# JiehongLin/SAM-6D

Hardware: AMD Instinct MI355X
Metric: RGB-D frames/sec (SAM-6D per-frame hot path: SAM ViT-H encoder + ISM scoring + PEM) (higher is better)
Workload: dtype bf16 (SAM ViT-H: 87 % of the step) + f16 (PEM ViT-B feature extractor) + f32 (ISM scoring, PEM point transformer and pose solvers); 1 GPU; LM-O single object: 32 frames/step/GPU, 640x480 RGB-D -> 1024^2 SAM input, P=128 proposals x 42 templates (scored in groups of 8 frames), 1 instance/frame, 2048 pts (PEM batch 32); sam_frames_per_launch_group=16, pem_vit_dtype=fp16 (set by bench.py; the library default is fp32)

## Files before the change

sam6d_amd/csrc/s6d_attn_win16.h:

```cpp
#pragma once
#include "s6d_attn_common.h"

namespace S6D_ATTN_NS {

#ifndef S6D_WIN16_STREAM
#define S6D_WIN16_STREAM 1
#endif
#ifndef S6D_WIN16_KSWZ
#define S6D_WIN16_KSWZ 1
#endif

template <int HD>
struct RelFrags {
  union { uint4 u; bf16x8 v; } rh[2][Cfg<HD>::KS], rw[2][Cfg<HD>::KS];
  __device__ __forceinline__ void load(const AttnParams &p, int lane) {
    using C = Cfg<HD>;
    const int g = lane >> 4, c = lane & 15;
#pragma unroll
    for (int jt = 0; jt < 2; ++jt)
#pragma unroll
      for (int ks = 0; ks < C::KS; ++ks) {
        rh[jt][ks].u = *reinterpret_cast<const uint4 *>(p.rel_h + (size_t)(jt * 16 + c) * C::HDP + ks * 32 + g * 8);
        rw[jt][ks].u = *reinterpret_cast<const uint4 *>(p.rel_w + (size_t)(jt * 16 + c) * C::HDP + ks * 32 + g * 8);
      }
  }
};

constexpr int W16_LT = 36;

template <int HD, int NR, int SRC>
__device__ __forceinline__ void win16_tables(const RelFrags<HD> &rf, int S, int qy0, int rstride,
                                             const bf16x8 (*qf)[Cfg<HD>::KS], float *tab, float (*twr)[4],
                                             float (*thv)[16], int lane) {
  using C = Cfg<HD>;
  const int g = lane >> 4, c = lane & 15;
#pragma unroll
  for (int n = 0; n < NR; ++n) {
    const int qy = min(qy0 + n * rstride, S - 1);
    f32x4 ah[2], aw[2];
#pragma unroll
    for (int jt = 0; jt < 2; ++jt) {
      ah[jt] = f32x4{0.f, 0.f, 0.f, 0.f};
      aw[jt] = f32x4{0.f, 0.f, 0.f, 0.f};
#pragma unroll
      for (int ks = 0; ks < C::KS; ++ks) {
        aw[jt] = S6D_ATTN_MFMA16(rf.rw[jt][ks].v, qf[n][ks], aw[jt]);
        ah[jt] = S6D_ATTN_MFMA16(rf.rh[jt][ks].v, qf[n][ks], ah[jt]);
      }
    }
#pragma unroll
    for (int jt = 0; jt < 2; ++jt)
      *reinterpret_cast<float4 *>(tab + c * W16_LT + jt * 16 + g * 4) =
          make_float4(aw[jt][0] * kLog2e, aw[jt][1] * kLog2e, aw[jt][2] * kLog2e, aw[jt][3] * kLog2e);
    S6D_WAVE_RENDEZVOUS();
#pragma unroll
    for (int r = 0; r < 4; ++r) {
      const int kx = g * 4 + r;
      const float v = tab[c * W16_LT + min(max(c - kx + S - 1, 0), 31)];
      twr[n][r] = (kx < S && c < S) ? v : -1e30f;
    }
    S6D_WAVE_RENDEZVOUS();
#pragma unroll
    for (int jt = 0; jt < 2; ++jt)
      *reinterpret_cast<float4 *>(tab + c * W16_LT + jt * 16 + g * 4) =
          make_float4(ah[jt][0] * kLog2e, ah[jt][1] * kLog2e, ah[jt][2] * kLog2e, ah[jt][3] * kLog2e);
    S6D_WAVE_RENDEZVOUS();
#pragma unroll
    for (int ky = 0; ky < SRC; ++ky) {
      const float v = tab[c * W16_LT + min(max(qy - ky + S - 1, 0), 31)];
      thv[n][ky] = ky < S ? v : -1e30f;
    }
    S6D_WAVE_RENDEZVOUS();
  }
}

struct Win16NoMid {
  __device__ __forceinline__ void operator()() const {}
};
template <int HD, int NS, int SRC, bool EXACT, int KROWT = Cfg<HD>::KROW, bool KSWZ = false, class MID = Win16NoMid>
__device__ __forceinline__ void win16_pass(const AttnParams &p, const u16 *Kl, const u16 *Vl, int S, int SR, int b,
                                           int wy, int wx, int head, int qy0, int rstride,
                                           const bf16x8 (&qf)[NS][Cfg<HD>::KS], const float (*twr)[4],
                                           const float (*thv)[16], int lane, MID mid = MID()) {
  using C = Cfg<HD>;
  const int g = lane >> 4, c = lane & 15;
  const int Cc = p.nh * HD;
  float sp[NS][SRC][4], m[NS];
#pragma unroll
  for (int n = 0; n < NS; ++n) m[n] = -1e29f;
  f32x4 cb[NS];
  {
    const float inv = 1.0f / p.scale_log2;
#pragma unroll
    for (int n = 0; n < NS; ++n)
#pragma unroll
      for (int r = 0; r < 4; ++r) cb[n][r] = twr[n][r] * inv;
  }
  bf16x8 kf[2][C::KS];
  const int gk = KSWZ ? (g ^ kswz(c)) : g;
  auto kload = [&](int ky, bf16x8 (&dst)[C::KS]) {
    const int kyc = EXACT ? ky : min(ky, SR - 1);
#pragma unroll
    for (int ks = 0; ks < C::KS; ++ks) {
      dst[ks] = *reinterpret_cast<const bf16x8 *>(Kl + (kyc * 16 + c) * KROWT + ks * 32 + gk * 8);
      if (KROWT < C::HDP && ks * 32 + 32 > HD && ks * 32 + g * 8 >= HD) {
        union { bf16x8 v; uint4 u; } z;
        z.u = make_uint4(0, 0, 0, 0);
        dst[ks] = z.v;
      }
    }
  };
  kload(0, kf[0]);
#pragma unroll
  for (int ky = 0; ky < SRC; ++ky) {
    if (ky + 1 < SRC) kload(ky + 1, kf[(ky + 1) & 1]);
    f32x4 acc[NS];
#pragma unroll
    for (int n = 0; n < NS; ++n) acc[n] = cb[n];
#pragma unroll
    for (int ks = 0; ks < C::KS; ++ks)
#pragma unroll
      for (int n = 0; n < NS; ++n)
        acc[n] = S6D_ATTN_MFMA16(kf[ky & 1][ks], qf[n][ks], acc[n]);
#pragma unroll
    for (int n = 0; n < NS; ++n) {
#pragma unroll
      for (int r = 0; r < 4; ++r) sp[n][ky][r] = acc[n][r];
      const float mk = __builtin_fmaf(fmaxf(fmaxf(acc[n][0], acc[n][1]), fmaxf(acc[n][2], acc[n][3])), p.scale_log2, thv[n][ky]);
      m[n] = fmaxf(m[n], mk);
    }
  }
#pragma unroll
  for (int n = 0; n < NS; ++n) {
    m[n] = fmaxf(m[n], __shfl_xor(m[n], 16));
    m[n] = fmaxf(m[n], __shfl_xor(m[n], 32));
  }
  f32x4 oacc[NS][C::DT], lacc[NS];
#pragma unroll
  for (int n = 0; n < NS; ++n) {
    lacc[n] = f32x4{0.f, 0.f, 0.f, 0.f};
#pragma unroll
    for (int dt = 0; dt < C::DT; ++dt) oacc[n][dt] = f32x4{0.f, 0.f, 0.f, 0.f};
  }
  union { bf16x8 v; u16 hh[8]; } ones;
#pragma unroll
  for (int i = 0; i < 8; ++i) ones.hh[i] = S6D_ATTN_ONE;
#pragma unroll
  for (int u = 0; u < SRC; u += 2) {
    if (u == ((SRC / 2 + 1) & ~1)) {
      __builtin_amdgcn_sched_barrier(0);
      mid();
      __builtin_amdgcn_sched_barrier(0);
    }
    if (EXACT || u < SR) {
      union { bf16x8 v; s16x4 q[2]; } va[C::DT];
      const u16 *vrow = Vl + (u * 16 + g * 4 + (c >> 2)) * C::VROW + (c & 3) * 4;
#pragma unroll
      for (int dt = 0; dt < C::DT; ++dt) {
        va[dt].q[0] = __builtin_amdgcn_ds_read_tr16_b64_v4i16((S6D_LDS(s16x4) *)(vrow + dt * 16));
        va[dt].q[1] = __builtin_amdgcn_ds_read_tr16_b64_v4i16((S6D_LDS(s16x4) *)(vrow + 16 * C::VROW + dt * 16));
      }
      union { bf16x8 v; u16 hh[8]; } pb[NS];
#pragma unroll
      for (int n = 0; n < NS; ++n)
#pragma unroll
        for (int h = 0; h < 2; ++h) {
          const float nb = thv[n][u + h] - m[n];
          for (int r = 0; r < 4; ++r) pb[n].hh[h * 4 + r] = f2bf(fast_exp2(__builtin_fmaf(sp[n][u + h][r], p.scale_log2, nb)));
        }
#pragma unroll
      for (int n = 0; n < NS; ++n) lacc[n] = S6D_ATTN_MFMA16(ones.v, pb[n].v, lacc[n]);
#pragma unroll
      for (int dt = 0; dt < C::DT; ++dt)
#pragma unroll
        for (int n = 0; n < NS; ++n)
          oacc[n][dt] = S6D_ATTN_MFMA16(va[dt].v, pb[n].v, oacc[n][dt]);
    }
  }
#pragma unroll
  for (int n = 0; n < NS; ++n) {
    const int qy = qy0 + n * rstride;
    const int y = wy * p.ws + qy, x = wx * p.ws + c;
    if ((qy < S) && c < S && (y < p.H) && (x < p.W)) {
      const float inv = 1.0f / lacc[n][0];
      u16 *dst = p.out + ((size_t)(b * p.H + y) * p.W + x) * (size_t)Cc + head * HD;
#pragma unroll
      for (int dt = 0; dt < C::DT; ++dt) {
        union { uint2 u2; u16 hh[4]; } o;
#pragma unroll
        for (int r = 0; r < 4; ++r) o.hh[r] = f2bf(oacc[n][dt][r] * inv);
        *reinterpret_cast<uint2 *>(dst + dt * 16 + g * 4) = o.u2;
      }
    }
  }
}

template <int HD, int SRC, int KROWT, bool KSWZ, class NEXTQ, class THISQ>
__device__ __forceinline__ void win16_pass_stream(const AttnParams &p, const u16 *Kl, const u16 *Vl, int S, int b, int wy, int wx,
                                                  int head, int qy0, int rstride, const bf16x8 (&qf)[2][Cfg<HD>::KS],
                                                  const float (*twr)[4], const float (*thv)[16], int lane, NEXTQ next_q, THISQ this_q) {
  using C = Cfg<HD>;
  constexpr int NS = 2;
  static_assert(SRC % 2 == 0 && SRC >= 4, "whole 32-key steps");
  const int g = lane >> 4, c = lane & 15;
  const int Cc = p.nh * HD;
  const int gk = KSWZ ? (g ^ kswz(c)) : g;
  f32x4 cb[NS];
  {
    const float inv = 1.0f / p.scale_log2;
#pragma unroll
    for (int n = 0; n < NS; ++n)
#pragma unroll
      for (int r = 0; r < 4; ++r) cb[n][r] = twr[n][r] * inv;
  }
  bf16x8 kf[2][C::KS];
  auto kload = [&](int ky, bf16x8 (&dst)[C::KS]) __attribute__((always_inline)) {
#pragma unroll
    for (int ks = 0; ks < C::KS; ++ks) {
      dst[ks] = *reinterpret_cast<const bf16x8 *>(Kl + (ky * 16 + c) * KROWT + ks * 32 + gk * 8);
      if (KROWT < C::HDP && ks * 32 + 32 > HD && ks * 32 + g * 8 >= HD) {
        union { bf16x8 v; uint4 u; } z;
        z.u = make_uint4(0, 0, 0, 0);
        dst[ks] = z.v;
      }
    }
  };
  auto scores = [&](const bf16x8 (&k)[C::KS], f32x4 (&acc)[NS]) __attribute__((always_inline)) {
#pragma unroll
    for (int n = 0; n < NS; ++n) acc[n] = cb[n];
#pragma unroll
    for (int ks = 0; ks < C::KS; ++ks)
#pragma unroll
      for (int n = 0; n < NS; ++n) acc[n] = S6D_ATTN_MFMA16(k[ks], qf[n][ks], acc[n]);
  };
  f32x4 s0[NS], s1[NS];
  kload(0, kf[0]);
  kload(1, kf[1]);
  scores(kf[0], s0);
  scores(kf[1], s1);
  float m[NS];
#pragma unroll
  for (int n = 0; n < NS; ++n) {
    const float m0 = __builtin_fmaf(fmaxf(fmaxf(s0[n][0], s0[n][1]), fmaxf(s0[n][2], s0[n][3])), p.scale_log2, thv[n][0]);
    const float m1 = __builtin_fmaf(fmaxf(fmaxf(s1[n][0], s1[n][1]), fmaxf(s1[n][2], s1[n][3])), p.scale_log2, thv[n][1]);
    float v = fmaxf(fmaxf(m0, m1), -1e29f);
    v = fmaxf(v, __shfl_xor(v, 16));
    v = fmaxf(v, __shfl_xor(v, 32));
    m[n] = v;
  }
  union { bf16x8 v; u16 hh[8]; } ones;
#pragma unroll
  for (int i = 0; i < 8; ++i) ones.hh[i] = S6D_ATTN_ONE;
  f32x4 oacc[NS][C::DT], lacc[NS];
  int round = 0;
  for (;;) {
#pragma unroll
    for (int n = 0; n < NS; ++n) {
      lacc[n] = f32x4{0.f, 0.f, 0.f, 0.f};
#pragma unroll
      for (int dt = 0; dt < C::DT; ++dt) oacc[n][dt] = f32x4{0.f, 0.f, 0.f, 0.f};
    }
#pragma unroll
    for (int u = 0; u < SRC; u += 2) {
      if (u > 0 || round > 0) {
        kload(u, kf[0]);
        kload(u + 1, kf[1]);
        scores(kf[0], s0);
        scores(kf[1], s1);
      }
      if (u == SRC - 2 && round == 0) {
        __builtin_amdgcn_sched_barrier(0);
        next_q();
        __builtin_amdgcn_sched_barrier(0);
      }
      union { bf16x8 v; s16x4 q[2]; } va[C::DT];
      const u16 *vrow = Vl + (u * 16 + g * 4 + (c >> 2)) * C::VROW + (c & 3) * 4;
#pragma unroll
      for (int dt = 0; dt < C::DT; ++dt) {
        va[dt].q[0] = __builtin_amdgcn_ds_read_tr16_b64_v4i16((S6D_LDS(s16x4) *)(vrow + dt * 16));
        va[dt].q[1] = __builtin_amdgcn_ds_read_tr16_b64_v4i16((S6D_LDS(s16x4) *)(vrow + 16 * C::VROW + dt * 16));
      }
      union { bf16x8 v; u16 hh[8]; } pb[NS];
#pragma unroll
      for (int n = 0; n < NS; ++n) {
        const float nb0 = thv[n][u] - m[n], nb1 = thv[n][u + 1] - m[n];
#pragma unroll
        for (int r = 0; r < 4; ++r) {
          pb[n].hh[r] = f2bf(fast_exp2(__builtin_fmaf(s0[n][r], p.scale_log2, nb0)));
          pb[n].hh[4 + r] = f2bf(fast_exp2(__builtin_fmaf(s1[n][r], p.scale_log2, nb1)));
        }
      }
#pragma unroll
      for (int n = 0; n < NS; ++n) lacc[n] = S6D_ATTN_MFMA16(ones.v, pb[n].v, lacc[n]);
#pragma unroll
      for (int dt = 0; dt < C::DT; ++dt)
#pragma unroll
        for (int n = 0; n < NS; ++n) oacc[n][dt] = S6D_ATTN_MFMA16(va[dt].v, pb[n].v, oacc[n][dt]);
    }
    bool any_bad = false;
#pragma unroll
    for (int n = 0; n < NS; ++n) {
      const int qy = qy0 + n * rstride;
      int ovf = 0;
#pragma unroll
      for (int dt = 0; dt < C::DT; ++dt)
#pragma unroll
        for (int r = 0; r < 4; ++r) ovf |= !(fabsf(oacc[n][dt][r]) < kNoMaxFinite);
      ovf |= __shfl_xor(ovf, 16);
      ovf |= __shfl_xor(ovf, 32);
      const bool bad = (qy < S) && (c < S) && (!(lacc[n][0] < kNoMaxSumLimit) || ovf);
      m[n] = bad ? m[n] + 96.0f : m[n];
      any_bad |= bad;
    }
    if (!__any(any_bad) || round >= 40) break;
    if (round == 0) this_q();
    ++round;
  }
  if (round > 0) next_q();
#pragma unroll
  for (int n = 0; n < NS; ++n) {
    const int qy = qy0 + n * rstride;
    const int y = wy * p.ws + qy, x = wx * p.ws + c;
    if ((qy < S) && c < S && (y < p.H) && (x < p.W)) {
      const float inv = 1.0f / lacc[n][0];
      u16 *dst = p.out + ((size_t)(b * p.H + y) * p.W + x) * (size_t)Cc + head * HD;
#pragma unroll
      for (int dt = 0; dt < C::DT; ++dt) {
        union { uint2 u2; u16 hh[4]; } o;
#pragma unroll
        for (int r = 0; r < 4; ++r) o.hh[r] = f2bf(oacc[n][dt][r] * inv);
        *reinterpret_cast<uint2 *>(dst + dt * 16 + g * 4) = o.u2;
      }
    }
  }
}

template <int HD, int WAVES>
__global__ __launch_bounds__(WAVES * 64) void attn_window16_kernel(AttnParams p) {
  using C = Cfg<HD>;
  S6D_DYN_LDS(smem);
  const int S = p.S, SR = (S + 1) & ~1;
  u16 *Kl = reinterpret_cast<u16 *>(smem);
  u16 *Vl = Kl + (size_t)SR * 16 * C::KROW;
  float *tabs = reinterpret_cast<float *>(Vl + (size_t)SR * 16 * C::VROW);
  const int tid = threadIdx.x, wave = tid >> 6, lane = tid & 63;
  const int g = lane >> 4, c = lane & 15;
  float *tab = tabs + (size_t)wave * 16 * W16_LT;

  WinItem item;
  item.decode(p, blockIdx.x);
  const int head = item.head, wx = item.wx, wy = item.wy, b = item.b;
  const int Cc = p.nh * HD;
  constexpr int MAXROWS = 2;
  static_assert(2 * WAVES >= 16, "two rows per wave must cover 16 query rows");
  bf16x8 qfa[MAXROWS][C::KS];
#pragma unroll
  for (int i = 0; i < MAXROWS; ++i) {
    const int qy = wave + i * WAVES;
    const int y = wy * p.ws + qy, x = wx * p.ws + c;
    const bool qwin = c < S && qy < S, qimg = qwin && (y < p.H) && (x < p.W);
#pragma unroll
    for (int ks = 0; ks < C::KS; ++ks) {
      union { uint4 u; bf16x8 v; } t;
      const int d0 = ks * 32 + g * 8;
      const int dc = d0 < HD ? d0 : HD - 8;
      const size_t tokc = (size_t)(b * p.H + min(y, p.H - 1)) * p.W + min(x, p.W - 1);
      const u16 *src = qimg ? qkv_at(p, tokc, 0, head) + dc : p.qkv_bias + head * HD + dc;
      t.u = *reinterpret_cast<const uint4 *>(src);
      if (!(qwin && d0 < HD)) t.u = make_uint4(0, 0, 0, 0);
      qfa[i][ks] = t.v;
    }
  }
  RelFrags<HD> rf;
  rf.load(p, lane);
  constexpr int UN = 10;
  const int total = SR * 16 * (C::KPARTS + C::VPARTS);
  uint4 sv[UN];
  u16 *sdst[UN];
  auto issue = [&](int i0) {
#pragma unroll
    for (int n = 0; n < UN; ++n) {
      const int i = i0 + n * WAVES * 64;
      const int iq = min(i, total - 1);
      const bool isv = iq >= SR * 16 * C::KPARTS;
      const int ii = isv ? iq - SR * 16 * C::KPARTS : iq;
      const int parts = isv ? C::VPARTS : C::KPARTS;
      const int slot = ii / parts, part = ii - slot * parts;
      const int ky = slot >> 4, kx = slot & 15;
      const int y = wy * p.ws + ky, x = wx * p.ws + kx;
      sdst[n] = (i < total) ? (isv ? Vl + slot * C::VROW + part * 8 : Kl + slot * C::KROW + part * 8) : nullptr;
      const bool img = (y < p.H) && (x < p.W);
      const int dc = part * 8 < HD ? part * 8 : HD - 8;
      const size_t tokc = (size_t)(b * p.H + min(y, p.H - 1)) * p.W + min(x, p.W - 1);
      const int sel = (isv ? 2 : 1) * Cc + head * HD + dc;
      const u16 *src = img ? qkv_at(p, tokc, isv ? 2 : 1, head) + dc : p.qkv_bias + sel;
      sv[n] = *reinterpret_cast<const uint4 *>(src);
      if (!(ky < S && kx < S && part * 8 < HD)) sv[n] = make_uint4(0, 0, 0, 0);
    }
  };
  auto commit = [&]() {
#pragma unroll
    for (int n = 0; n < UN; ++n)
      if (sdst[n]) *reinterpret_cast<uint4 *>(sdst[n]) = sv[n];
  };
  const bool stage = !(kAbl & 1);
  if (stage) issue(tid);
  float twr[MAXROWS][4], thv[MAXROWS][16];
  if (!(kAbl & 2)) {
    if (S > WAVES) {
      if (S == 14)
        win16_tables<HD, 2, 14>(rf, S, wave, WAVES, qfa, tab, twr, thv, lane);
      else
        win16_tables<HD, 2, 16>(rf, S, wave, WAVES, qfa, tab, twr, thv, lane);
    } else if (wave < S) {
      win16_tables<HD, 1, 8>(rf, S, wave, WAVES, qfa, tab, twr, thv, lane);
    }
  }
  if (stage) {
    commit();
    for (int i0 = tid + UN * WAVES * 64; i0 < total; i0 += UN * WAVES * 64) {
      issue(i0);
      commit();
    }
  }
  __syncthreads();

  if (S <= WAVES) {
    if (wave < S && !(kAbl & 2)) {
      const bf16x8 (&q1)[1][C::KS] = reinterpret_cast<const bf16x8 (&)[1][C::KS]>(qfa[0]);
      win16_pass<HD, 1, 8, false>(p, Kl, Vl, S, SR, b, wy, wx, head, wave, WAVES, q1, twr, thv, lane);
    }
  } else if (!(kAbl & 2)) {
    static_assert(MAXROWS >= 2 || WAVES >= 16, "row bookkeeping");
    const bf16x8 (&q2)[2][C::KS] = reinterpret_cast<const bf16x8 (&)[2][C::KS]>(qfa[0]);
    if (S == 14) {
      win16_pass<HD, 2, 14, true>(p, Kl, Vl, S, SR, b, wy, wx, head, wave, WAVES, q2, twr, thv, lane);
    } else
      win16_pass<HD, 2, 16, false>(p, Kl, Vl, S, SR, b, wy, wx, head, wave, WAVES, q2, twr, thv, lane);
  }
}


template <int HD, bool S14>
__global__ __launch_bounds__(512) void attn_window16p_kernel(AttnParams p, int nitems) {
  using C = Cfg<HD>;
  constexpr int WAVES = 8;
  constexpr int KROWT = HD + 8, KCH = KROWT / 8, VCH = C::VROW / 8;
  S6D_DYN_LDS(smem);
  const int S = p.S, SR = (S + 1) & ~1;
  const int kchunks = SR * 16 * KCH, vchunks = SR * 16 * VCH;
  const int kinstr = (kchunks + 63) >> 6, vinstr = (vchunks + 63) >> 6;
  const int kbytes = kinstr << 10, bufbytes = kbytes + (vinstr << 10);
  u16 *relh = reinterpret_cast<u16 *>(smem + 2 * bufbytes);
  u16 *relw = relh + 32 * C::HDP;
  const int tid = threadIdx.x, wave = __builtin_amdgcn_readfirstlane(tid >> 6), lane = tid & 63;
  const int g = lane >> 4, c = lane & 15;
  const int Cc = p.nh * HD;
  constexpr int RCH = C::HDP / 8;
  for (int i = tid; i < 2 * 32 * RCH; i += 512) {
    const bool w = i >= 32 * RCH;
    const int ii = w ? i - 32 * RCH : i;
    const int row = ii / RCH, ch = ii - row * RCH;
    reinterpret_cast<uint4 *>(w ? relw : relh)[row * RCH + (ch ^ ((row >> 2) & 3))] = reinterpret_cast<const uint4 *>(w ? p.rel_w : p.rel_h)[ii];
  }

  constexpr int MAXI = S14 ? 5 : 6;
  static_assert(((S14 ? 14 : 16) * 16 * (KCH > VCH ? KCH : VCH) + 63) / 64 <= WAVES * MAXI,
                "attn_window16p_kernel: K / V image has more DMA pieces than the unrolled slots (raise MAXI)");
  unsigned kvc[MAXI];
  {
#pragma unroll
    for (int i = 0; i < MAXI; ++i) {
      unsigned both = 0;
#pragma unroll
      for (int which = 1; which <= 2; ++which) {
        const int rowch = which == 1 ? KCH : VCH, nch = which == 1 ? kchunks : vchunks;
        const int k = wave + i * WAVES;
        const int j = min((k << 6) + lane, nch - 1);
        const int slot = j / rowch, pp = j - slot * rowch;
        const int ky = slot >> 4, kx = slot & 15;
        const int part = (S6D_WIN16_KSWZ && which == 1 && pp * 8 < HD) ? pp ^ kswz(kx) : pp;
        const bool inwin = ky < S && kx < S && part * 8 < HD;
        const unsigned v = (unsigned)(ky & 15) | ((unsigned)kx << 4) | ((unsigned)part << 8) | ((unsigned)inwin << 12);
        both |= which == 1 ? v : v << 16;
      }
      kvc[i] = both;
    }
  }
  auto stage_image = [&](const WinItem &it, int which, char *dst_base) __attribute__((always_inline)) {
    const int ninstr = which == 1 ? kinstr : vinstr;
    const int y0 = it.wy * p.ws, x0 = it.wx * p.ws, bH = it.b * p.H;
    const u16 *base = qkv_at(p, 0, which, it.head);
    const u16 *bias_base = p.qkv_bias + which * Cc + it.head * HD;
#pragma unroll
    for (int i = 0; i < MAXI; ++i) {
      const int k = wave + i * WAVES;
      if (k < ninstr) {
        unsigned cc = which == 1 ? kvc[i] : kvc[i] >> 16;
        S6D_PIN(cc);
        const int ky = (int)(cc & 15u), kx = (int)((cc >> 4) & 15u), po = min((int)((cc >> 8) & 15u) * 8, HD - 8);
        const int y = y0 + ky, x = x0 + kx;
        const bool img = (y < p.H) && (x < p.W);
        const unsigned tok = (unsigned)(bH + min(y, p.H - 1)) * (unsigned)p.W + (unsigned)min(x, p.W - 1);
        const u16 *s_img = base + (size_t)tok * (size_t)p.tok_stride + po;
        const u16 *src = img ? s_img : bias_base + po;
        const void *sp = (cc >> 12) & 1u ? (const void *)src : (const void *)&g_attn_zero16;
        S6D_LDS(char) *dst = (S6D_LDS(char) *)dst_base + (k << 10);
        lds_dma16_m0(sp, dst);
      }
    }
  };
  constexpr int MAXROWS = 2;
  bf16x8 qfa[MAXROWS][C::KS];
  auto load_q = [&](const WinItem &it, bool raw, bf16x8 (&qdst)[MAXROWS][C::KS]) __attribute__((always_inline)) {
#pragma unroll
    for (int i = 0; i < MAXROWS; ++i) {
      const int qy = wave + i * WAVES;
      const int y = it.wy * p.ws + qy, x = it.wx * p.ws + c;
      const bool qwin = c < S && qy < S, qimg = qwin && (y < p.H) && (x < p.W);
#pragma unroll
      for (int ks = 0; ks < C::KS; ++ks) {
        union { uint4 u; bf16x8 v; } t;
        const int d0 = ks * 32 + g * 8;
        const int dc = d0 < HD ? d0 : HD - 8;
        const size_t tokc = (size_t)(it.b * p.H + min(y, p.H - 1)) * p.W + min(x, p.W - 1);
        const u16 *src = qimg ? qkv_at(p, tokc, 0, it.head) + dc : p.qkv_bias + it.head * HD + dc;
        t.u = *reinterpret_cast<const uint4 *>(src);
        if (!raw && !(qwin && d0 < HD)) t.u = make_uint4(0, 0, 0, 0);
        qdst[i][ks] = t.v;
      }
    }
  };
  auto mask_q = [&]() __attribute__((always_inline)) {
#pragma unroll
    for (int i = 0; i < MAXROWS; ++i) {
      const bool qwin = c < S && wave + i * WAVES < S;
#pragma unroll
      for (int ks = 0; ks < C::KS; ++ks) {
        union { uint4 u; bf16x8 v; } t;
        t.v = qfa[i][ks];
        if (!(qwin && ks * 32 + g * 8 < HD)) t.u = make_uint4(0, 0, 0, 0);
        qfa[i][ks] = t.v;
      }
    }
  };

  WinItem cur, nxt;
  int id = blockIdx.x;
  cur.decode(p, id);
  load_q(cur, false, qfa);
  stage_image(cur, 1, smem);
  stage_image(cur, 2, smem + kbytes);
  S6D_VMCNT(0);
  __syncthreads();
  int buf = 0;
  long long wtk[8] = {0, 0, 0, 0, 0, 0, 0, 0}, wsum[6] = {0, 0, 0, 0, 0, 0};
  for (; id < nitems; id += gridDim.x) {
    char *cb = smem + buf * bufbytes, *nb = smem + (buf ^ 1) * bufbytes;
    const bool more = id + (int)gridDim.x < nitems;
    S6D_TICK(wtk, 0);
    if (more) {
      nxt.decode(p, id + gridDim.x);
      stage_image(nxt, 1, nb);
    }
    float twr[MAXROWS][4], thv[MAXROWS][16];
    {
      RelFrags<HD> rf;
#pragma unroll
      for (int jt = 0; jt < 2; ++jt)
#pragma unroll
        for (int ks = 0; ks < C::KS; ++ks) {
          const int ro = (jt * 16 + c) * C::HDP + ((ks * 4 + g) ^ (((jt * 16 + c) >> 2) & 3)) * 8;
          rf.rh[jt][ks].u = *reinterpret_cast<const uint4 *>(relh + ro);
          rf.rw[jt][ks].u = *reinterpret_cast<const uint4 *>(relw + ro);
        }
      float *tab = reinterpret_cast<float *>(nb + kbytes) + (size_t)wave * 16 * W16_LT;
      if (S == 14)
        win16_tables<HD, 2, 14>(rf, S, wave, WAVES, qfa, tab, twr, thv, lane);
      else
        win16_tables<HD, 2, 16>(rf, S, wave, WAVES, qfa, tab, twr, thv, lane);
    }
    S6D_TICK(wtk, 1);
    __builtin_amdgcn_s_barrier();
    S6D_TICK(wtk, 2);
    if (more) stage_image(nxt, 2, nb + kbytes);
    S6D_TICK(wtk, 3);
    const u16 *Kl = reinterpret_cast<const u16 *>(cb), *Vl = reinterpret_cast<const u16 *>(cb + kbytes);
    const bf16x8 (&q2)[2][C::KS] = reinterpret_cast<const bf16x8 (&)[2][C::KS]>(qfa[0]);
    if (S14 && S6D_WIN16_STREAM) {
      auto next_q = [&]() __attribute__((always_inline)) {
        if (more) load_q(nxt, true, qfa);
      };
      auto this_q = [&]() __attribute__((always_inline)) { load_q(cur, false, qfa); };
      win16_pass_stream<HD, 14, KROWT, S6D_WIN16_KSWZ != 0>(p, Kl, Vl, S, cur.b, cur.wy, cur.wx, cur.head, wave, WAVES, q2, twr, thv, lane,
                                                            next_q, this_q);
    } else {
      auto mid = [&]() __attribute__((always_inline)) {
        if (more) load_q(nxt, true, qfa);
      };
      if (S14)
        win16_pass<HD, 2, 14, true, KROWT, S6D_WIN16_KSWZ != 0>(p, Kl, Vl, S, SR, cur.b, cur.wy, cur.wx, cur.head, wave, WAVES, q2, twr, thv, lane, mid);
      else
        win16_pass<HD, 2, 16, false, KROWT, S6D_WIN16_KSWZ != 0>(p, Kl, Vl, S, SR, cur.b, cur.wy, cur.wx, cur.head, wave, WAVES, q2, twr, thv, lane, mid);
    }
    S6D_TICK(wtk, 4);
    S6D_VMCNT(0);
    S6D_TICK(wtk, 5);
    __syncthreads();
    S6D_TICK(wtk, 6);
    if (S6D_G64_TIMING)
#pragma unroll
      for (int i = 0; i < 6; ++i) wsum[i] += wtk[i + 1] - wtk[i];
    mask_q();
    cur = nxt;
    buf ^= 1;
  }
  if (S6D_G64_TIMING && blockIdx.x == 8 && lane == 0) {
    long long *dbg = reinterpret_cast<long long *>(p.out + (size_t)p.B * p.H * p.W * p.nh * HD);
#pragma unroll
    for (int i = 0; i < 6; ++i) dbg[wave * 6 + i] = wsum[i];
  }
}

template <int HD>
static int launch_win16(AttnParams p, hipStream_t st) {
  using C = Cfg<HD>;
  constexpr int WAVES = 8;
  const int SR = (p.S + 1) & ~1;
  if (p.S > WAVES) {
    const int kin = (SR * 16 * (HD + 8) / 8 + 63) / 64, vin = (SR * 16 * C::VROW / 8 + 63) / 64;
    const size_t lds = (size_t)2 * (kin + vin) * 1024 + (size_t)2 * 32 * C::HDP * 2;
    const int nitems = p.B * p.nwy * p.nwx * p.nh;
    if (lds <= 160 * 1024 && (size_t)WAVES * 16 * W16_LT * 4 <= (size_t)vin * 1024) {
      int grid = nitems < 256 ? nitems : 256;
      if (s6d::g_s6d_persistent_grid_limit > 0 && s6d::g_s6d_persistent_grid_limit < grid) grid = s6d::g_s6d_persistent_grid_limit;
      if (grid >= 8) grid &= ~7;
      if (p.S == 14) {
        launch_lds(attn_window16p_kernel<HD, true>, grid, 512, lds, st, p, nitems);
      } else {
        launch_lds(attn_window16p_kernel<HD, false>, grid, 512, lds, st, p, nitems);
      }
      return launch_status();
    }
  }
  const size_t lds = (size_t)SR * 16 * (C::KROW + C::VROW) * 2 + (size_t)WAVES * 16 * W16_LT * 4;
  if (lds > 160 * 1024) return S6D_EUNSUPPORTED;
  launch_lds(attn_window16_kernel<HD, WAVES>, (unsigned)(p.B * p.nwy * p.nwx * p.nh), WAVES * 64, lds, st, p);
  return launch_status();
}

}
```

sam6d_amd/csrc/s6d_mem.h:

```cpp
#pragma once
#include <hip/hip_runtime.h>

#define S6D_LDS(T) __attribute__((address_space(3))) T
#define S6D_GLOBAL(T) __attribute__((address_space(1))) T
#ifdef HIPEMU
#define S6D_CONST(T) T
#else
#define S6D_CONST(T) __attribute__((address_space(4))) T
#endif

#ifdef HIPEMU
#define S6D_VMCNT(n) hipemu::vmcnt_wait(n)
#define S6D_LGKM0() do { } while (0)
#else
#define S6D_VMCNT(n) asm volatile("s_waitcnt vmcnt(" #n ")" ::: "memory")
#define S6D_LGKM0() asm volatile("s_waitcnt lgkmcnt(0)" ::: "memory")
#endif

#ifdef HIPEMU
#define S6D_PIN(x) do { } while (0)
#else
#define S6D_PIN(x) asm volatile("" : "+v"(x))
#endif

#ifdef HIPEMU
namespace s6d {
alignas(64) inline char emu_dyn_lds[160 * 1024];
}
#define S6D_DYN_LDS(name) static char (&name)[sizeof(::s6d::emu_dyn_lds)] = ::s6d::emu_dyn_lds
#else
#define S6D_DYN_LDS(name) extern __shared__ __attribute__((aligned(16))) char name[]
#endif

namespace s6d {

__device__ __forceinline__ void lds_dma16(const void *src, S6D_LDS(char) *dst) {
  __builtin_amdgcn_global_load_lds((const S6D_GLOBAL(void) *)src, dst, 16, 0, 0);
}

__device__ __forceinline__ void lds_dma16_m0(const void *src, S6D_LDS(char) *dst) {
#ifdef HIPEMU
  lds_dma16(src, dst);
#else
  const unsigned a = __builtin_amdgcn_readfirstlane((unsigned)(size_t)dst);
  asm volatile("s_mov_b32 m0, %1\n\ts_nop 0\n\tglobal_load_lds_dwordx4 %0, off" ::"v"(src), "s"(a) : "memory", "m0");
#endif
}

}
```

Baseline: 168.4 frames/s.

## Use scalar-base 32-bit offset LDS DMA for S=14 window attention staging

For the S=14 persistent windowed attention kernel, K/V staging now uses a scalar base pointer plus per-lane 32-bit offsets, with exec-masked skipping of padding chunks. Those padding chunks are pre-zeroed in LDS instead of being loaded from a global zero buffer. Interior windows take a fast path with no per-lane boundary clamping, Q loads use precomputed offsets, and the output store is factored into a helper. The aim is to cut VALU address arithmetic and wasted DMA traffic. In exchange it needs an extra lgkmcnt wait and a re-zero of the scratch region, and it is gated on strides that fit in 32-bit offsets.

```diff
diff --git a/sam6d_amd/csrc/s6d_attn_win16.h b/sam6d_amd/csrc/s6d_attn_win16.h
--- a/sam6d_amd/csrc/s6d_attn_win16.h
+++ b/sam6d_amd/csrc/s6d_attn_win16.h
@@ -1,4 +1,6 @@
 #pragma once
+#include <type_traits>
+
 #include "s6d_attn_common.h"
 
 namespace S6D_ATTN_NS {
@@ -71,6 +73,31 @@
       thv[n][ky] = ky < S ? v : -1e30f;
     }
     S6D_WAVE_RENDEZVOUS();
+  }
+}
+
+template <int HD, int NS>
+__device__ __forceinline__ void win16_store_rows(const AttnParams &p, int S, int b, int wy, int wx, int head, int qy0, int rstride, int lane,
+                                                 const f32x4 (&oacc)[NS][Cfg<HD>::DT], const f32x4 (&lacc)[NS]) {
+  using C = Cfg<HD>;
+  const int g = lane >> 4, c = lane & 15;
+  const int Cc = p.nh * HD, x0 = wx * p.ws;
+#pragma unroll
+  for (int n = 0; n < NS; ++n) {
+    const int qy = qy0 + n * rstride;
+    const int y = wy * p.ws + qy;
+    if ((qy < S) && (y < p.H) && c < min(S, p.W - x0)) {
+      const float inv = 1.0f / lacc[n][0];
+      u16 *row = p.out + ((size_t)(b * p.H + y) * p.W + x0) * (size_t)Cc + head * HD;
+      u16 *dst = reinterpret_cast<u16 *>(reinterpret_cast<char *>(row) + ((unsigned)c * (unsigned)Cc) * 2u);
+#pragma unroll
+      for (int dt = 0; dt < C::DT; ++dt) {
+        union { uint2 u2; u16 hh[4]; } o;
+#pragma unroll
+        for (int r = 0; r < 4; ++r) o.hh[r] = f2bf(oacc[n][dt][r] * inv);
+        *reinterpret_cast<uint2 *>(dst + dt * 16 + g * 4) = o.u2;
+      }
+    }
   }
 }
 
@@ -203,7 +230,6 @@
   constexpr int NS = 2;
   static_assert(SRC % 2 == 0 && SRC >= 4, "whole 32-key steps");
   const int g = lane >> 4, c = lane & 15;
-  const int Cc = p.nh * HD;
   const int gk = KSWZ ? (g ^ kswz(c)) : g;
   f32x4 cb[NS];
   {
@@ -317,22 +343,7 @@
     ++round;
   }
   if (round > 0) next_q();
-#pragma unroll
-  for (int n = 0; n < NS; ++n) {
-    const int qy = qy0 + n * rstride;
-    const int y = wy * p.ws + qy, x = wx * p.ws + c;
-    if ((qy < S) && c < S && (y < p.H) && (x < p.W)) {
-      const float inv = 1.0f / lacc[n][0];
-      u16 *dst = p.out + ((size_t)(b * p.H + y) * p.W + x) * (size_t)Cc + head * HD;
-#pragma unroll
-      for (int dt = 0; dt < C::DT; ++dt) {
-        union { uint2 u2; u16 hh[4]; } o;
-#pragma unroll
-        for (int r = 0; r < 4; ++r) o.hh[r] = f2bf(oacc[n][dt][r] * inv);
-        *reinterpret_cast<uint2 *>(dst + dt * 16 + g * 4) = o.u2;
-      }
-    }
-  }
+  win16_store_rows<HD, NS>(p, S, b, wy, wx, head, qy0, rstride, lane, oacc, lacc);
 }
 
 template <int HD, int WAVES>
@@ -447,13 +458,13 @@
   constexpr int WAVES = 8;
   constexpr int KROWT = HD + 8, KCH = KROWT / 8, VCH = C::VROW / 8;
   S6D_DYN_LDS(smem);
-  const int S = p.S, SR = (S + 1) & ~1;
+  const int S = S14 ? 14 : p.S, SR = (S + 1) & ~1;
   const int kchunks = SR * 16 * KCH, vchunks = SR * 16 * VCH;
   const int kinstr = (kchunks + 63) >> 6, vinstr = (vchunks + 63) >> 6;
   const int kbytes = kinstr << 10, bufbytes = kbytes + (vinstr << 10);
   u16 *relh = reinterpret_cast<u16 *>(smem + 2 * bufbytes);
   u16 *relw = relh + 32 * C::HDP;
-  const int tid = threadIdx.x, wave = __builtin_amdgcn_readfirstlane(tid >> 6), lane = tid & 63;
+  const int tid = threadIdx.x, wave = __builtin_amdgcn_readfirstlane(tid >> 6) & (WAVES - 1), lane = tid & 63;
   const int g = lane >> 4, c = lane & 15;
   const int Cc = p.nh * HD;
   constexpr int RCH = C::HDP / 8;
@@ -487,47 +498,138 @@
       kvc[i] = both;
     }
   }
+  const unsigned w16 = (unsigned)p.W & 0xffffu, tokb = ((unsigned)p.tok_stride * 2u) & 0xffffffu;
+  auto chunk_off = [&](unsigned cc) __attribute__((always_inline)) {
+    return ((cc & 15u) * w16 + ((cc >> 4) & 15u)) * tokb + ((cc >> 4) & 0xf0u);
+  };
+  auto zero_chunks = [&](int which, char *dst_base, bool scratch_only) __attribute__((always_inline)) {
+    const int ninstr = which == 1 ? kinstr : vinstr;
+#pragma unroll
+    for (int i = 0; i < MAXI; ++i) {
+      const int k = wave + i * WAVES;
+      if (k < ninstr && (!scratch_only || (k << 10) < WAVES * 16 * W16_LT * 4)) {
+        unsigned cc = which == 1 ? kvc[i] : kvc[i] >> 16;
+        S6D_PIN(cc);
+        if (!((cc >> 12) & 1u)) *reinterpret_cast<uint4 *>(dst_base + (k << 10) + lane * 16) = make_uint4(0, 0, 0, 0);
+      }
+    }
+  };
+  if (S14) {
+#pragma unroll
+    for (int b2 = 0; b2 < 2; ++b2) {
+      zero_chunks(1, smem + b2 * bufbytes, false);
+      zero_chunks(2, smem + b2 * bufbytes + kbytes, false);
+    }
+  }
   auto stage_image = [&](const WinItem &it, int which, char *dst_base) __attribute__((always_inline)) {
     const int ninstr = which == 1 ? kinstr : vinstr;
-    const int y0 = it.wy * p.ws, x0 = it.wx * p.ws, bH = it.b * p.H;
-    const u16 *base = qkv_at(p, 0, which, it.head);
-    const u16 *bias_base = p.qkv_bias + which * Cc + it.head * HD;
-#pragma unroll
-    for (int i = 0; i < MAXI; ++i) {
-      const int k = wave + i * WAVES;
-      if (k < ninstr) {
-        unsigned cc = which == 1 ? kvc[i] : kvc[i] >> 16;
-        S6D_PIN(cc);
-        const int ky = (int)(cc & 15u), kx = (int)((cc >> 4) & 15u), po = min((int)((cc >> 8) & 15u) * 8, HD - 8);
-        const int y = y0 + ky, x = x0 + kx;
-        const bool img = (y < p.H) && (x < p.W);
-        const unsigned tok = (unsigned)(bH + min(y, p.H - 1)) * (unsigned)p.W + (unsigned)min(x, p.W - 1);
-        const u16 *s_img = base + (size_t)tok * (size_t)p.tok_stride + po;
-        const u16 *src = img ? s_img : bias_base + po;
-        const void *sp = (cc >> 12) & 1u ? (const void *)src : (const void *)&g_attn_zero16;
-        S6D_LDS(char) *dst = (S6D_LDS(char) *)dst_base + (k << 10);
-        lds_dma16_m0(sp, dst);
+    const int y0 = it.wy * p.ws, x0 = it.wx * p.ws;
+    const char *bias_base = reinterpret_cast<const char *>(p.qkv_bias + which * Cc + it.head * HD);
+    if constexpr (S14) {
+      const int vy = p.H - y0, vx = p.W - x0;
+      const char *base = reinterpret_cast<const char *>(qkv_at(p, (size_t)(it.b * p.H + y0) * p.W + x0, which, it.head));
+      unsigned wpiece = (unsigned)wave << 10;
+      S6D_PIN_S(wpiece);
+      if (vy >= S && vx >= S) {
+#pragma unroll
+        for (int i = 0; i < MAXI; ++i) {
+          const int k = wave + i * WAVES;
+          if (k < ninstr) {
+            unsigned cc = which == 1 ? kvc[i] : kvc[i] >> 16;
+            S6D_PIN(cc);
+            lds_dma16_sbase(base, (cc >> 12) & 1u ? chunk_off(cc) : kLdsDmaSkip, (S6D_LDS(char) *)dst_base + (wpiece + (i << 13)));
+          }
+        }
+      } else {
+#pragma unroll
+        for (int i = 0; i < MAXI; ++i) {
+          const int k = wave + i * WAVES;
+          if (k < ninstr) {
+            unsigned cc = which == 1 ? kvc[i] : kvc[i] >> 16;
+            S6D_PIN(cc);
+            const bool img = (int)(cc & 15u) < vy && (int)((cc >> 4) & 15u) < vx;
+            const char *src = img ? base + chunk_off(cc) : bias_base + ((cc >> 4) & 0xf0u);
+            const void *sp = (cc >> 12) & 1u ? (const void *)src : (const void *)&g_attn_zero16;
+            lds_dma16_m0(sp, (S6D_LDS(char) *)dst_base + (wpiece + (i << 13)));
+          }
+        }
+      }
+    } else {
+      const int bH = it.b * p.H;
+      const u16 *base = qkv_at(p, 0, which, it.head);
+#pragma unroll
+      for (int i = 0; i < MAXI; ++i) {
+        const int k = wave + i * WAVES;
+        if (k < ninstr) {
+          unsigned cc = which == 1 ? kvc[i] : kvc[i] >> 16;
+          S6D_PIN(cc);
+          const int ky = (int)(cc & 15u), kx = (int)((cc >> 4) & 15u), po = min((int)((cc >> 8) & 15u) * 8, HD - 8);
+          const int y = y0 + ky, x = x0 + kx;
+          const bool img = (y < p.H) && (x < p.W);
+          const unsigned tok = (unsigned)(bH + min(y, p.H - 1)) * (unsigned)p.W + (unsigned)min(x, p.W - 1);
+          const u16 *s_img = base + (size_t)tok * (size_t)p.tok_stride + po;
+          const u16 *src = img ? s_img : reinterpret_cast<const u16 *>(bias_base) + po;
+          const void *sp = (cc >> 12) & 1u ? (const void *)src : (const void *)&g_attn_zero16;
+          lds_dma16_m0(sp, (S6D_LDS(char) *)dst_base + (k << 10));
+        }
       }
     }
   };
   constexpr int MAXROWS = 2;
   bf16x8 qfa[MAXROWS][C::KS];
+  const int cq = min(c, S - 1);
+  const unsigned qoff = ((unsigned)cq * (unsigned)p.tok_stride + (unsigned)(g * 8)) * 2u;
+  const unsigned qoff_last = ((unsigned)cq * (unsigned)p.tok_stride + (unsigned)min((C::KS - 1) * 32 + g * 8, HD - 8)) * 2u;
   auto load_q = [&](const WinItem &it, bool raw, bf16x8 (&qdst)[MAXROWS][C::KS]) __attribute__((always_inline)) {
-#pragma unroll
-    for (int i = 0; i < MAXROWS; ++i) {
-      const int qy = wave + i * WAVES;
-      const int y = it.wy * p.ws + qy, x = it.wx * p.ws + c;
-      const bool qwin = c < S && qy < S, qimg = qwin && (y < p.H) && (x < p.W);
-#pragma unroll
-      for (int ks = 0; ks < C::KS; ++ks) {
-        union { uint4 u; bf16x8 v; } t;
-        const int d0 = ks * 32 + g * 8;
-        const int dc = d0 < HD ? d0 : HD - 8;
-        const size_t tokc = (size_t)(it.b * p.H + min(y, p.H - 1)) * p.W + min(x, p.W - 1);
-        const u16 *src = qimg ? qkv_at(p, tokc, 0, it.head) + dc : p.qkv_bias + it.head * HD + dc;
-        t.u = *reinterpret_cast<const uint4 *>(src);
-        if (!raw && !(qwin && d0 < HD)) t.u = make_uint4(0, 0, 0, 0);
-        qdst[i][ks] = t.v;
+    if constexpr (S14) {
+      const int y0 = it.wy * p.ws, x0 = it.wx * p.ws;
+      const int vy = p.H - y0, vx = p.W - x0;
+      union { uint4 u; bf16x8 v; } t[MAXROWS][C::KS];
+      auto rows = [&](auto interior) __attribute__((always_inline)) {
+#pragma unroll
+        for (int i = 0; i < MAXROWS; ++i) {
+          const int qyc = min(wave + i * WAVES, S - 1);
+          const char *base = reinterpret_cast<const char *>(qkv_at(p, (size_t)(it.b * p.H + min(y0 + qyc, p.H - 1)) * p.W + x0, 0, it.head));
+          const char *bias_base = reinterpret_cast<const char *>(p.qkv_bias + it.head * HD);
+          const bool qimg = qyc < vy && cq < vx;
+#pragma unroll
+          for (int ks = 0; ks < C::KS; ++ks) {
+            const unsigned off = ks * 32 + 32 <= HD ? qoff + ks * 64 : qoff_last;
+            const int dc = min(ks * 32 + g * 8, HD - 8);
+            t[i][ks].u = *reinterpret_cast<const uint4 *>(decltype(interior)::value || qimg ? base + off : bias_base + dc * 2);
+          }
+        }
+      };
+      if (vy >= S && vx >= S)
+        rows(std::true_type());
+      else
+        rows(std::false_type());
+#pragma unroll
+      for (int i = 0; i < MAXROWS; ++i) {
+        const bool qwin = c < S && wave + i * WAVES < S;
+#pragma unroll
+        for (int ks = 0; ks < C::KS; ++ks) {
+          if (!raw && !(qwin && ks * 32 + g * 8 < HD)) t[i][ks].u = make_uint4(0, 0, 0, 0);
+          qdst[i][ks] = t[i][ks].v;
+        }
+      }
+    } else {
+#pragma unroll
+      for (int i = 0; i < MAXROWS; ++i) {
+        const int qy = wave + i * WAVES;
+        const int y = it.wy * p.ws + qy, x = it.wx * p.ws + c;
+        const bool qwin = c < S && qy < S, qimg = qwin && (y < p.H) && (x < p.W);
+#pragma unroll
+        for (int ks = 0; ks < C::KS; ++ks) {
+          union { uint4 u; bf16x8 v; } t;
+          const int d0 = ks * 32 + g * 8;
+          const int dc = d0 < HD ? d0 : HD - 8;
+          const size_t tokc = (size_t)(it.b * p.H + min(y, p.H - 1)) * p.W + min(x, p.W - 1);
+          const u16 *src = qimg ? qkv_at(p, tokc, 0, it.head) + dc : p.qkv_bias + it.head * HD + dc;
+          t.u = *reinterpret_cast<const uint4 *>(src);
+          if (!raw && !(qwin && d0 < HD)) t.u = make_uint4(0, 0, 0, 0);
+          qdst[i][ks] = t.v;
+        }
       }
     }
   };
@@ -581,9 +683,13 @@
         win16_tables<HD, 2, 16>(rf, S, wave, WAVES, qfa, tab, twr, thv, lane);
     }
     S6D_TICK(wtk, 1);
+    if (S14) S6D_LGKM0();
     __builtin_amdgcn_s_barrier();
     S6D_TICK(wtk, 2);
-    if (more) stage_image(nxt, 2, nb + kbytes);
+    if (more) {
+      if (S14) zero_chunks(2, nb + kbytes, true);
+      stage_image(nxt, 2, nb + kbytes);
+    }
     S6D_TICK(wtk, 3);
     const u16 *Kl = reinterpret_cast<const u16 *>(cb), *Vl = reinterpret_cast<const u16 *>(cb + kbytes);
     const bf16x8 (&q2)[2][C::KS] = reinterpret_cast<const bf16x8 (&)[2][C::KS]>(qfa[0]);
@@ -631,7 +737,8 @@
     const int kin = (SR * 16 * (HD + 8) / 8 + 63) / 64, vin = (SR * 16 * C::VROW / 8 + 63) / 64;
     const size_t lds = (size_t)2 * (kin + vin) * 1024 + (size_t)2 * 32 * C::HDP * 2;
     const int nitems = p.B * p.nwy * p.nwx * p.nh;
-    if (lds <= 160 * 1024 && (size_t)WAVES * 16 * W16_LT * 4 <= (size_t)vin * 1024) {
+    const bool off32 = p.tok_stride > 0 && p.tok_stride < (1l << 22) && p.W < (1 << 16) && (unsigned long long)(16 * p.W) * (unsigned long long)p.tok_stride * 2 < (1ull << 31);
+    if (lds <= 160 * 1024 && (size_t)WAVES * 16 * W16_LT * 4 <= (size_t)vin * 1024 && off32) {
       int grid = nitems < 256 ? nitems : 256;
       if (s6d::g_s6d_persistent_grid_limit > 0 && s6d::g_s6d_persistent_grid_limit < grid) grid = s6d::g_s6d_persistent_grid_limit;
       if (grid >= 8) grid &= ~7;
diff --git a/sam6d_amd/csrc/s6d_mem.h b/sam6d_amd/csrc/s6d_mem.h
--- a/sam6d_amd/csrc/s6d_mem.h
+++ b/sam6d_amd/csrc/s6d_mem.h
@@ -19,8 +19,10 @@
 
 #ifdef HIPEMU
 #define S6D_PIN(x) do { } while (0)
+#define S6D_PIN_S(x) do { } while (0)
 #else
 #define S6D_PIN(x) asm volatile("" : "+v"(x))
+#define S6D_PIN_S(x) asm volatile("" : "+s"(x))
 #endif
 
 #ifdef HIPEMU
@@ -47,4 +49,28 @@
 #endif
 }
 
+constexpr unsigned kLdsDmaSkip = 0xffffffffu;
+__device__ __forceinline__ void lds_dma16_sbase(const void *base, unsigned off, S6D_LDS(char) *dst) {
+#ifdef HIPEMU
+  const unsigned long long d = (unsigned long long)(uintptr_t)(void *)dst;
+  const bool on = off != kLdsDmaSkip;
+  hipemu::begin_exchange(d, 8);
+  for (int k = 0; k < 64; ++k)
+    if (k < hipemu::g_blk->w_alive[hipemu::wave_of()] && hipemu::peek<unsigned long long>(k) != d) {
+      std::fprintf(stderr, "hipemu: lds_dma16_sbase with a lane-dependent LDS base\n");
+      std::abort();
+    }
+  hipemu::end_exchange();
+  hipemu::glds_issue(on ? (const void *)((const char *)base + off) : base, (char *)(void *)dst + hipemu::lane_of() * 16, on ? 16 : 0);
+#else
+  const unsigned a = __builtin_amdgcn_readfirstlane((unsigned)(size_t)dst);
+  unsigned long long keep;
+  asm volatile("v_cmp_ne_u32_e32 vcc, -1, %1\n\ts_and_saveexec_b64 %0, vcc\n\ts_mov_b32 m0, %3\n\ts_nop 0\n\t"
+               "global_load_lds_dwordx4 %1, %2\n\ts_mov_b64 exec, %0"
+               : "=&s"(keep)
+               : "v"(off), "s"(base), "s"(a)
+               : "memory", "m0", "vcc");
+#endif
 }
+
+}
```

Result: no change. 168.5 frames/s (median of 3 runs) (+0.1%).
